# FitSNAP/FitSNAP

Hardware: AMD Instinct MI355X
Metric: training rows/sec through A^T A + solve, 1000000 x 128 fp64 in total over the GPUs (strong scaling) (higher is better)
Workload: dtype f64

## Files before the change

fitsnap_amd/csrc/fsnap_condest.h:

```cpp
#pragma once

#include <cmath>
#include <cstdint>
#include <vector>

namespace fsnap {

struct CondEstimate {
    double lambda_min = 0.0;
    int steps = 0;
};

inline double tridiag_lambda_max(const double* a, const double* b, int n) {
    double lo = a[0], hi = a[0];
    for (int i = 0; i < n; ++i) {
        const double r = (i > 0 ? std::fabs(b[i - 1]) : 0.0) + (i + 1 < n ? std::fabs(b[i]) : 0.0);
        if (a[i] - r < lo) lo = a[i] - r;
        if (a[i] + r > hi) hi = a[i] + r;
    }
    if (n == 1) return a[0];
    for (int it = 0; it < 200 && hi - lo > 4.0e-16 * std::fmax(std::fabs(hi), std::fabs(lo)); ++it) {
        const double x = 0.5 * (lo + hi);
        int above = 0;
        double d = 1.0;
        for (int i = 0; i < n; ++i) {
            const double off = i > 0 ? b[i - 1] * b[i - 1] : 0.0;
            d = (a[i] - x) - (i > 0 ? off / d : 0.0);
            if (d == 0.0) d = -1.0e-300;
            if (d > 0.0) ++above;
        }
        if (above > 0) lo = x; else hi = x;
    }
    return 0.5 * (lo + hi);
}

template <class ApplyInv>
CondEstimate lanczos_lambda_min(int n, ApplyInv&& apply_inv, int min_steps = 2, int max_steps = 8, double growth = 1.25,
                                double* theta_trace = nullptr) {
    CondEstimate out;
    if (n <= 0) return out;
    if (max_steps > 16) max_steps = 16;
    if (theta_trace)
        for (int j = 0; j < max_steps; ++j) theta_trace[j] = 0.0;
    std::vector<double> V((size_t)(max_steps + 1) * n), w(n);
    double al[16], be[16];
    uint64_t s = 0x9E3779B97F4A7C15ull;
    double nrm = 0.0;
    for (int i = 0; i < n; ++i) {
        s = s * 6364136223846793005ull + 1442695040888963407ull;
        const double u = (double)(int64_t)(s >> 11) * (1.0 / 9007199254740992.0);
        const double v = (u < 0.5 ? -1.0 : 1.0) * (0.25 + 0.75 * std::fabs(2.0 * u - 1.0));
        V[i] = v;
        nrm += v * v;
    }
    nrm = 1.0 / std::sqrt(nrm);
    for (int i = 0; i < n; ++i) V[i] *= nrm;
    double theta_prev = 0.0, theta = 0.0;
    for (int j = 0; j < max_steps; ++j) {
        double* vj = V.data() + (size_t)j * n;
        for (int i = 0; i < n; ++i) w[i] = vj[i];
        if (!apply_inv(w.data())) return CondEstimate{0.0, j + 1};
        double a = 0.0, chk = 0.0;
        for (int i = 0; i < n; ++i) {
            a += vj[i] * w[i];
            chk += w[i] * 0.0;
        }
        if (chk != 0.0 || !(a > 0.0)) return CondEstimate{0.0, j + 1};
        al[j] = a;
        out.steps = j + 1;
        theta = tridiag_lambda_max(al, be, j + 1);
        if (!(theta > 0.0) || !std::isfinite(theta)) return CondEstimate{0.0, j + 1};
        if (theta_trace) theta_trace[j] = theta;
        if (j + 1 >= min_steps && theta <= growth * theta_prev) break;
        if (j + 1 == max_steps) break;
        theta_prev = theta;
        for (int pass = 0; pass < 2; ++pass)
            for (int p = 0; p <= j; ++p) {
                const double* vp = V.data() + (size_t)p * n;
                double d = 0.0;
                for (int i = 0; i < n; ++i) d += vp[i] * w[i];
                for (int i = 0; i < n; ++i) w[i] -= d * vp[i];
            }
        double b = 0.0;
        for (int i = 0; i < n; ++i) b += w[i] * w[i];
        b = std::sqrt(b);
        if (!(b > 1.0e-14 * theta)) break;
        be[j] = b;
        double* vn = V.data() + (size_t)(j + 1) * n;
        const double ib = 1.0 / b;
        for (int i = 0; i < n; ++i) vn[i] = w[i] * ib;
    }
    out.lambda_min = 1.0 / theta;
    return out;
}

}
```

fitsnap_amd/csrc/fsnap_solve.cpp:

```cpp
#include <atomic>
#include <chrono>
#include <cstdio>
#include <cmath>
#include <cstdlib>
#include <cstdint>
#include <cstring>
#include <limits>
#include <mutex>
#include <thread>
#include <vector>

#include "../../include/fsnap_hip.h"
#include "fsnap_condest.h"

static thread_local double g_cond_info[4] = {0.0, 0.0, 0.0, 0.0};

extern "C" __attribute__((visibility("hidden"))) void fsnap_cond_note(double min_pivot, double lambda_min, int steps, int where) {
    g_cond_info[0] = min_pivot;
    g_cond_info[1] = lambda_min;
    g_cond_info[2] = (double)steps;
    g_cond_info[3] = (double)where;
}

extern "C" int fsnap_cond_info(double* info) {
// ... 155 lines not shown
    for (int c0 = ((je >> 5) + first_chunk) << 5; c0 < n; c0 += 32 * chunk_step) {
        const int cw = (n - c0 < 32) ? n - c0 : 32;
        const int i_end = (c0 + 32 < n) ? c0 + 32 : n;
        int i = je;
        if (cw == 32) {
            for (; i + 4 <= i_end; i += 4) {
                double* r0 = a + (size_t)i * n + c0;
                double* r1 = r0 + n;
                double* r2 = r1 + n;
                double* r3 = r2 + n;
                v8d y00 = *(const v8du*)(r0), y01 = *(const v8du*)(r0 + 8), y02 = *(const v8du*)(r0 + 16), y03 = *(const v8du*)(r0 + 24);
                v8d y10 = *(const v8du*)(r1), y11 = *(const v8du*)(r1 + 8), y12 = *(const v8du*)(r1 + 16), y13 = *(const v8du*)(r1 + 24);
                v8d y20 = *(const v8du*)(r2), y21 = *(const v8du*)(r2 + 8), y22 = *(const v8du*)(r2 + 16), y23 = *(const v8du*)(r2 + 24);
                v8d y30 = *(const v8du*)(r3), y31 = *(const v8du*)(r3 + 8), y32 = *(const v8du*)(r3 + 16), y33 = *(const v8du*)(r3 + 24);
                const double* uk = a + (size_t)jb * n;
                for (int k = 0; k < nk; ++k, uk += n) {
                    const v8d u0 = *(const v8du*)(uk + c0), u1 = *(const v8du*)(uk + c0 + 8);
                    const v8d u2 = *(const v8du*)(uk + c0 + 16), u3 = *(const v8du*)(uk + c0 + 24);
                    const double f0 = uk[i], f1 = uk[i + 1], f2 = uk[i + 2], f3 = uk[i + 3];
                    const v8d b0 = {f0, f0, f0, f0, f0, f0, f0, f0}, b1 = {f1, f1, f1, f1, f1, f1, f1, f1};
                    const v8d b2 = {f2, f2, f2, f2, f2, f2, f2, f2}, b3 = {f3, f3, f3, f3, f3, f3, f3, f3};
                    y00 -= b0 * u0; y01 -= b0 * u1; y02 -= b0 * u2; y03 -= b0 * u3;
                    y10 -= b1 * u0; y11 -= b1 * u1; y12 -= b1 * u2; y13 -= b1 * u3;
                    y20 -= b2 * u0; y21 -= b2 * u1; y22 -= b2 * u2; y23 -= b2 * u3;
                    y30 -= b3 * u0; y31 -= b3 * u1; y32 -= b3 * u2; y33 -= b3 * u3;
                }
                *(v8du*)(r0) = y00; *(v8du*)(r0 + 8) = y01; *(v8du*)(r0 + 16) = y02; *(v8du*)(r0 + 24) = y03;
                *(v8du*)(r1) = y10; *(v8du*)(r1 + 8) = y11; *(v8du*)(r1 + 16) = y12; *(v8du*)(r1 + 24) = y13;
                *(v8du*)(r2) = y20; *(v8du*)(r2 + 8) = y21; *(v8du*)(r2 + 16) = y22; *(v8du*)(r2 + 24) = y23;
                *(v8du*)(r3) = y30; *(v8du*)(r3 + 8) = y31; *(v8du*)(r3 + 16) = y32; *(v8du*)(r3 + 24) = y33;
            }
        }
        if (cw == 16) {
            for (; i + 4 <= i_end; i += 4) {
                double* r0 = a + (size_t)i * n + c0;
                double* r1 = r0 + n;
                double* r2 = r1 + n;
                double* r3 = r2 + n;
                v8d y00 = *(const v8du*)(r0), y01 = *(const v8du*)(r0 + 8);
                v8d y10 = *(const v8du*)(r1), y11 = *(const v8du*)(r1 + 8);
                v8d y20 = *(const v8du*)(r2), y21 = *(const v8du*)(r2 + 8);
                v8d y30 = *(const v8du*)(r3), y31 = *(const v8du*)(r3 + 8);
                const double* uk = a + (size_t)jb * n;
                for (int k = 0; k < nk; ++k, uk += n) {
                    const v8d u0 = *(const v8du*)(uk + c0), u1 = *(const v8du*)(uk + c0 + 8);
                    const double f0 = uk[i], f1 = uk[i + 1], f2 = uk[i + 2], f3 = uk[i + 3];
                    const v8d b0 = {f0, f0, f0, f0, f0, f0, f0, f0}, b1 = {f1, f1, f1, f1, f1, f1, f1, f1};
                    const v8d b2 = {f2, f2, f2, f2, f2, f2, f2, f2}, b3 = {f3, f3, f3, f3, f3, f3, f3, f3};
                    y00 -= b0 * u0; y01 -= b0 * u1;
                    y10 -= b1 * u0; y11 -= b1 * u1;
                    y20 -= b2 * u0; y21 -= b2 * u1;
                    y30 -= b3 * u0; y31 -= b3 * u1;
                }
                *(v8du*)(r0) = y00; *(v8du*)(r0 + 8) = y01;
                *(v8du*)(r1) = y10; *(v8du*)(r1 + 8) = y11;
                *(v8du*)(r2) = y20; *(v8du*)(r2 + 8) = y21;
                *(v8du*)(r3) = y30; *(v8du*)(r3 + 8) = y31;
            }
        }
        for (; i < i_end; ++i) {
            double* ri = a + (size_t)i * n + c0;
            const double* uk = a + (size_t)jb * n;
            for (int k = 0; k < nk; ++k, uk += n) axpy_neg(ri, uk + c0, uk[i], cw);
        }
    }
}

int chol_upper_rb(double* a, int n, double* min_piv2, int NBK) {
    double mp = std::numeric_limits<double>::infinity();
    for (int jb = 0; jb < n; jb += NBK) {
        const int je = (jb + NBK < n) ? jb + NBK : n;
        const int fail = chol_panel(a, n, jb, je, &mp);
        if (fail >= 0) {
            if (min_piv2) *min_piv2 = mp;
            return fail;
        }
        if (je < n) chol_trailing_chunks(a, n, jb, je, 0, 1);
    }
    if (min_piv2) *min_piv2 = mp;
    return -1;
}

FSNAP_CLONES void chol_solve_inv(const double* u, int n, double* x, double* inv) {
    for (int k = 0; k < n; ++k) inv[k] = 1.0 / u[(size_t)k * n + k];
    for (int k = 0; k < n; ++k) {
        const double* r = u + (size_t)k * n;
        x[k] *= inv[k];
        axpy_neg(x + k + 1, r + k + 1, x[k], n - 1 - k);
    }
    for (int i = n - 1; i >= 0; --i) {
        const double* r = u + (size_t)i * n;
        x[i] = (x[i] - dotv(r + i + 1, x + i + 1, n - 1 - i)) * inv[i];
    }
}
void chol_solve(const double* u, int n, double* x) {
    static thread_local vec inv;
    inv.resize(n);
    chol_solve_inv(u, n, x, inv.data());
}


#define LD8(p) (*reinterpret_cast<const v8du*>(p))
#define ST8(p, v) (*reinterpret_cast<v8du*>(p) = (v))
#define BC8(f) (v8d{(f), (f), (f), (f), (f), (f), (f), (f)})

FSNAP_INLINE void prefetch_g_rows(const double* G, int K, int r0, int r1) {
    if (r1 > K) r1 = K;
    for (int i = r0; i < r1; ++i) {
        const double* gi = G + (size_t)i * K;
        for (int j = i & ~7; j < K; j += 8) __builtin_prefetch(gi + j, 0, 2);
    }
}

FSNAP_INLINE void scaled_row(const double* G, const double* dsc, int K, int Kp, int i, double alpha, bool upper_only,
                             double* U, v8d& chk0, v8d& chk1, double& chk) {
    const v8d zero = {0, 0, 0, 0, 0, 0, 0, 0};
    const double* gi = G + (size_t)i * K;
    double* ui = U + (size_t)i * Kp;
    const double di = dsc[i];
    const v8d dv = {di, di, di, di, di, di, di, di};
    const int j0 = i & ~7;
    int j = 0;
    for (; j + 8 <= j0; j += 8) *(v8du*)(ui + j) = zero;
    if (upper_only && j + 8 <= K) {
        typedef long long v8l __attribute__((vector_size(64)));
        const v8l lanes = {0, 1, 2, 3, 4, 5, 6, 7};
        const v8l keep = (lanes + (long long)j) >= (long long)i;
        const v8d g0 = (v8d)((v8l)(*(const v8du*)(gi + j)) & keep);
        chk0 += g0 * zero;
        *(v8du*)(ui + j) = g0 * dv * *(const v8du*)(dsc + j);
        j += 8;
    }
    for (; j + 16 <= K; j += 16) {
        const v8d g0 = *(const v8du*)(gi + j), g1 = *(const v8du*)(gi + j + 8);
        chk0 += g0 * zero;
        chk1 += g1 * zero;
        *(v8du*)(ui + j) = g0 * dv * *(const v8du*)(dsc + j);
        *(v8du*)(ui + j + 8) = g1 * dv * *(const v8du*)(dsc + j + 8);
    }
    for (; j + 8 <= K; j += 8) {
        const v8d g0 = *(const v8du*)(gi + j);
        chk0 += g0 * zero;
        *(v8du*)(ui + j) = g0 * dv * *(const v8du*)(dsc + j);
    }
    for (; j < K; ++j) {
        const double gij = (upper_only && j < i) ? 0.0 : gi[j];
        ui[j] = gij * di * dsc[j];
        chk += gij * 0.0;
    }
    for (; j < Kp; ++j) ui[j] = 0.0;
    ui[i] = (gi[i] + alpha) * di * di;
}

template <bool RHS>
FSNAP_INLINE void left_update_8x16(const double* u, int n, int jb, int c0, v8d (&y)[16], double* z) {
    v8d zv = {0, 0, 0, 0, 0, 0, 0, 0};
    if (RHS) zv = LD8(z + jb);
    const double* uk = u;
    for (int k = 0; k < jb; ++k, uk += n) {
        const v8d u0 = LD8(uk + c0), u1 = LD8(uk + c0 + 8);
        const double* f = uk + jb;
#pragma unroll
        for (int r = 0; r < 8; ++r) {
            const v8d b = BC8(f[r]);
            y[2 * r] -= b * u0;
            y[2 * r + 1] -= b * u1;
        }
        if (RHS) {
            const v8d zk = BC8(z[k]);
            zv -= zk * LD8(f);
        }
    }
    if (RHS) ST8(z + jb, zv);
}

FSNAP_INLINE int fused_diag_block(double* u, int n, int jb, double* z, double* inv, double* mp) {
    const int c0 = jb & ~15, off = jb - c0;
    double* blk = u + (size_t)jb * n + c0;
    if (jb > 0) {
        v8d y[16];
#pragma unroll
        for (int r = 0; r < 8; ++r) {
            y[2 * r] = LD8(blk + (size_t)r * n);
            y[2 * r + 1] = LD8(blk + (size_t)r * n + 8);
        }
        left_update_8x16<true>(u, n, jb, c0, y, z);
#pragma unroll
        for (int r = 0; r < 8; ++r) {
            ST8(blk + (size_t)r * n, y[2 * r]);
            ST8(blk + (size_t)r * n + 8, y[2 * r + 1]);
        }
    }
    for (int j = 0; j < 8; ++j) {
        double* uj = blk + (size_t)j * n;
        const double d = uj[off + j];
        if (d < *mp) *mp = d;
        if (!(d > 0.0) || !std::isfinite(d)) return jb + j;
        const double r = std::sqrt(d), iv = 1.0 / r;
        inv[j] = iv;
        const v8d ivv = BC8(iv);
        const v8d s0 = LD8(uj) * ivv, s1 = LD8(uj + 8) * ivv;
        ST8(uj, s0);
        ST8(uj + 8, s1);
        uj[off + j] = r;
        const double zj = z[jb + j] * iv;
        z[jb + j] = zj;
        for (int i = j + 1; i < 8; ++i) {
            const double f = uj[off + i];
            z[jb + i] -= zj * f;
            if (f != 0.0) {
                double* ui = blk + (size_t)i * n;
                const v8d fv = BC8(f);
                v8d y0 = LD8(ui), y1 = LD8(ui + 8);
                y0 -= fv * s0;
                y1 -= fv * s1;
                ST8(ui, y0);
                ST8(ui + 8, y1);
            }
        }
    }
    return -1;
}

FSNAP_INLINE void fused_right_block(double* u, int n, int jb, int c0, const double* inv) {
    double* blk = u + (size_t)jb * n + c0;
    v8d y[16];
#pragma unroll
    for (int r = 0; r < 8; ++r) {
        y[2 * r] = LD8(blk + (size_t)r * n);
        y[2 * r + 1] = LD8(blk + (size_t)r * n + 8);
    }
    left_update_8x16<false>(u, n, jb, c0, y, nullptr);
    const double* fr = u + (size_t)jb * n + jb;
#pragma unroll
    for (int j = 0; j < 8; ++j) {
        const v8d ivv = BC8(inv[j]);
        y[2 * j] *= ivv;
        y[2 * j + 1] *= ivv;
#pragma unroll
        for (int i = j + 1; i < 8; ++i) {
            const double f = fr[(size_t)j * n + i];
            if (f != 0.0) {
                const v8d fv = BC8(f);
                y[2 * i] -= fv * y[2 * j];
                y[2 * i + 1] -= fv * y[2 * j + 1];
            }
        }
    }
#pragma unroll
    for (int r = 0; r < 8; ++r) {
        ST8(blk + (size_t)r * n, y[2 * r]);
        ST8(blk + (size_t)r * n + 8, y[2 * r + 1]);
    }
}

FSNAP_CLONES int fused_scale_chol(const double* G, const double* dsc, int K, int Kp, double alpha, bool upper_only,
                                  double* u, double* z, double* inv, double* min_piv2, double* chk_out) {
    const v8d zero = {0, 0, 0, 0, 0, 0, 0, 0};
    v8d chk0 = zero, chk1 = zero;
    double chk = 0.0;
    double mp = std::numeric_limits<double>::infinity();
    int fail = -1;
    for (int jb = 0; jb < Kp && fail < 0; jb += 8) {
        prefetch_g_rows(G, K, jb + 16, jb + 24);
        for (int i = jb; i < jb + 8; ++i) {
            if (i < K) {
                scaled_row(G, dsc, K, Kp, i, alpha, upper_only, u, chk0, chk1, chk);
            } else {
                double* ui = u + (size_t)i * Kp;
                for (int j = 0; j < Kp; ++j) ui[j] = 0.0;
                ui[i] = 1.0;
            }
        }
        fail = fused_diag_block(u, Kp, jb, z, inv + jb, &mp);
        if (fail >= 0) break;
        for (int c0 = (jb & ~15) + 16; c0 < Kp; c0 += 16) fused_right_block(u, Kp, jb, c0, inv + jb);
    }
    const v8d cs = chk0 + chk1;
    chk += ((cs[0] + cs[1]) + (cs[2] + cs[3])) + ((cs[4] + cs[5]) + (cs[6] + cs[7]));
    *chk_out = chk;
    *min_piv2 = mp;
    return fail;
}

FSNAP_CLONES bool jacobi_scale(const double* d, int K, double alpha, double* dsc) {
    typedef long long v8l __attribute__((vector_size(64)));
    const v8d zero = {0, 0, 0, 0, 0, 0, 0, 0};
    const v8d av = BC8(alpha), one = BC8(1.0);
    v8l good = {-1, -1, -1, -1, -1, -1, -1, -1};
    int i = 0;
    for (; i + 8 <= K; i += 8) {
        const v8d g = LD8(d + i) + av;
        good &= (g > zero) & (g - g == zero);
        ST8(dsc + i, one / __builtin_elementwise_sqrt(g));
    }
    bool ok = (good[0] & good[1] & good[2] & good[3] & good[4] & good[5] & good[6] & good[7]) != 0;
    for (; i < K; ++i) {
        const double g = d[i] + alpha;
        if (!(g > 0.0) || !std::isfinite(g)) ok = false;
        dsc[i] = 1.0 / std::sqrt(g);
    }
    return ok;
}

FSNAP_CLONES void chol_back_inv(const double* u, int n, double* x, const double* inv) {
    for (int i = n - 1; i >= 0; --i) {
        const double* r = u + (size_t)i * n;
        x[i] = (x[i] - dotv(r + i + 1, x + i + 1, n - 1 - i)) * inv[i];
    }
}

bool lu_solve(double* a, int n, double* b) {
    std::vector<int> piv(n);
    for (int j = 0; j < n; ++j) {
        int p = j;
        double mx = std::fabs(a[(size_t)j * n + j]);
        for (int i = j + 1; i < n; ++i) {
            double v = std::fabs(a[(size_t)i * n + j]);
            if (v > mx) {
                mx = v;
                p = i;
            }
        }
        if (!(mx > 0.0) || !std::isfinite(mx)) return false;
        if (p != j) {
            for (int k = 0; k < n; ++k) std::swap(a[(size_t)j * n + k], a[(size_t)p * n + k]);
            std::swap(b[j], b[p]);
        }
        const double inv = 1.0 / a[(size_t)j * n + j];
        for (int i = j + 1; i < n; ++i) {
            double f = a[(size_t)i * n + j] * inv;
            if (f == 0.0) continue;
            a[(size_t)i * n + j] = f;
            for (int k = j + 1; k < n; ++k) a[(size_t)i * n + k] -= f * a[(size_t)j * n + k];
            b[i] -= f * b[j];
        }
    }
    for (int i = n - 1; i >= 0; --i) {
        double s = b[i];
        for (int k = i + 1; k < n; ++k) s -= a[(size_t)i * n + k] * b[k];
        b[i] = s / a[(size_t)i * n + i];
    }
    return true;
}

void jacobi_eigh(double* a, int n, double* eval, double* v) {
    for (int i = 0; i < n; ++i)
        for (int j = 0; j < n; ++j) v[(size_t)i * n + j] = (i == j) ? 1.0 : 0.0;
    for (int sweep = 0; sweep < 60; ++sweep) {
        double off = 0.0, diag = 0.0;
        for (int i = 0; i < n; ++i) {
            diag += a[(size_t)i * n + i] * a[(size_t)i * n + i];
            for (int j = i + 1; j < n; ++j) off += a[(size_t)i * n + j] * a[(size_t)i * n + j];
        }
        if (off == 0.0 || off <= 1e-34 * diag) break;
        for (int p = 0; p < n - 1; ++p) {
            for (int q = p + 1; q < n; ++q) {
                const double apq = a[(size_t)p * n + q];
                if (apq == 0.0) continue;
                const double app = a[(size_t)p * n + p], aqq = a[(size_t)q * n + q];
                if (std::fabs(apq) <= 1e-18 * std::sqrt(std::fabs(app) * std::fabs(aqq))) {
                    a[(size_t)p * n + q] = a[(size_t)q * n + p] = 0.0;
                    continue;
                }
                const double theta = (aqq - app) / (2.0 * apq);
                const double t = (theta >= 0 ? 1.0 : -1.0) / (std::fabs(theta) + std::sqrt(theta * theta + 1.0));
                const double cs = 1.0 / std::sqrt(t * t + 1.0), sn = t * cs;
                for (int k = 0; k < n; ++k) {
                    const double akp = a[(size_t)k * n + p], akq = a[(size_t)k * n + q];
                    a[(size_t)k * n + p] = cs * akp - sn * akq;
                    a[(size_t)k * n + q] = sn * akp + cs * akq;
                }
                for (int k = 0; k < n; ++k) {
                    const double apk = a[(size_t)p * n + k], aqk = a[(size_t)q * n + k];
                    a[(size_t)p * n + k] = cs * apk - sn * aqk;
                    a[(size_t)q * n + k] = sn * apk + cs * aqk;
                }
                a[(size_t)p * n + q] = a[(size_t)q * n + p] = 0.0;
                double* vp = v + (size_t)p * n;
                double* vq = v + (size_t)q * n;
                for (int k = 0; k < n; ++k) {
                    const double x = vp[k], y = vq[k];
                    vp[k] = cs * x - sn * y;
                    vq[k] = sn * x + cs * y;
                }
            }
        }
    }
    for (int i = 0; i < n; ++i) eval[i] = a[(size_t)i * n + i];
}

void residual_dot2(const double* M, int n, const double* x, const double* rhs, double* r) {
    for (int i = 0; i < n; ++i) {
        const double* mi = M + (size_t)i * n;
        v4d s = {0, 0, 0, 0}, c = {0, 0, 0, 0};
        int k = 0;
        for (; k + 4 <= n; k += 4) {
            const v4d a = ld4(mi + k), b = ld4(x + k);
            const v4d p = a * b;
            v4d e;
            for (int t = 0; t < 4; ++t) e[t] = __builtin_fma(a[t], b[t], -p[t]);
            const v4d sn = s + p;
            const v4d bp = sn - s;
            const v4d err = (s - (sn - bp)) + (p - bp);
            s = sn;
            c += err + e;
        }
        double ss = 0.0, cc = 0.0;
        for (int t = 0; t < 4; ++t) {
            const double sn = ss + s[t];
            const double bp = sn - ss;
            cc += (ss - (sn - bp)) + (s[t] - bp) + c[t];
            ss = sn;
        }
        for (; k < n; ++k) {
            const double p = mi[k] * x[k];
            const double e = __builtin_fma(mi[k], x[k], -p);
            const double sn = ss + p;
            const double bp = sn - ss;
            cc += (ss - (sn - bp)) + (p - bp) + e;
            ss = sn;
        }
        const double t1 = rhs[i] - ss;
        r[i] = t1 - cc;
    }
}

struct Reduced {
    int n;
    std::vector<int> idx;
    vec M;
    vec rhs;
};

bool all_finite(const double* p, size_t n) {
    const v8d zero = {0, 0, 0, 0, 0, 0, 0, 0};
    v8d s0 = zero, s1 = zero, s2 = zero, s3 = zero;
    size_t i = 0;
    for (; i + 32 <= n; i += 32) {
        s0 += *(const v8du*)(p + i) * zero;
        s1 += *(const v8du*)(p + i + 8) * zero;
        s2 += *(const v8du*)(p + i + 16) * zero;
        s3 += *(const v8du*)(p + i + 24) * zero;
    }
    const v8d s = (s0 + s1) + (s2 + s3);
    double t = ((s[0] + s[1]) + (s[2] + s[3])) + ((s[4] + s[5]) + (s[6] + s[7]));
    for (; i < n; ++i) t += p[i] * 0.0;
    return t == 0.0;
}

int scaled_chol_solve(const vec& M, const vec& rhs, int n, vec& x, double* min_piv2, fsnap::CondEstimate* cond = nullptr) {
    vec d(n), y(n);
    static thread_local vec S;
    S.resize((size_t)n * n);
    for (int i = 0; i < n; ++i) {
        const double g = M[(size_t)i * n + i];
        if (!(g > 0.0)) {
            if (min_piv2) *min_piv2 = 0.0;
            return i;
        }
        d[i] = 1.0 / std::sqrt(g);
// ... 23 lines not shown
    return -1;
}

int eig_pinv_solve(const vec& M, const vec& rhs, int n, double rel_cut, double shift, vec& x) {
    vec a(M), ev(n), V((size_t)n * n);
    jacobi_eigh(a.data(), n, ev.data(), V.data());
    double lmax = 0.0;
    for (int i = 0; i < n; ++i) lmax = std::fmax(lmax, std::fabs(ev[i]));
    x.assign(n, 0.0);
    int rank = 0;
    for (int i = 0; i < n; ++i) {
        if (!(ev[i] > rel_cut * lmax)) continue;
        ++rank;
        const double* vi = V.data() + (size_t)i * n;
        long double s = 0.0L;
        for (int k = 0; k < n; ++k) s += (long double)vi[k] * rhs[k];
        const double coef = (double)(s / (long double)(ev[i] + shift));
        for (int k = 0; k < n; ++k) x[k] += coef * vi[k];
    }
    return rank;
}

FSNAP_CLONES int chol_panel_diag(double* a, int n, int jb, int je, double* mp) {
    for (int j = jb; j < je; ++j) {
        double* uj = a + (size_t)j * n;
        const double d = uj[j];
        if (d < *mp) *mp = d;
        if (!(d > 0.0) || !std::isfinite(d)) return j;
        const double r = std::sqrt(d), inv = 1.0 / r;
        uj[j] = r;
        for (int k = j + 1; k < je; ++k) uj[k] *= inv;
        for (int i = j + 1; i < je; ++i) {
            const double f = uj[i];
            double* ui = a + (size_t)i * n;
            for (int k = i; k < je; ++k) ui[k] -= f * uj[k];
        }
    }
    return -1;
}
FSNAP_CLONES void chol_panel_tails(double* a, int n, int jb, int je, int first_chunk, int chunk_step) {
    for (int c0 = je + 32 * first_chunk; c0 < n; c0 += 32 * chunk_step) {
        const int cw = (n - c0 < 32) ? n - c0 : 32;
        for (int j = jb; j < je; ++j) {
            double* uj = a + (size_t)j * n;
            const double inv = 1.0 / uj[j];
            for (int k = 0; k < cw; ++k) uj[c0 + k] *= inv;
            for (int i = j + 1; i < je; ++i) axpy_neg(a + (size_t)i * n + c0, uj + c0, uj[i], cw);
        }
    }
}

int chol_upper_rb_mt(double* a, int n, double* min_piv2, int NBK, int nt) {
    struct Shared {
        std::atomic<int> arrived{0};
        std::atomic<int> phase{0};
        std::atomic<int> fail{-1};
        double mp = std::numeric_limits<double>::infinity();
    } sh;
    auto barrier = [&](int& local_phase) {
        ++local_phase;
        if (sh.arrived.fetch_add(1, std::memory_order_acq_rel) + 1 == nt) {
            sh.arrived.store(0, std::memory_order_relaxed);
            sh.phase.store(local_phase, std::memory_order_release);
        } else {
            int spins = 0;
            while (sh.phase.load(std::memory_order_acquire) != local_phase) {
#if defined(__x86_64__)
                __builtin_ia32_pause();
#endif
                if (++spins > 4096) {
                    std::this_thread::yield();
                    spins = 0;
                }
            }
        }
    };
    auto body = [&](int t) {
        int ph = 0;
        for (int jb = 0; jb < n; jb += NBK) {
            const int je = (jb + NBK < n) ? jb + NBK : n;
            if (t == 0) {
                const int f = chol_panel_diag(a, n, jb, je, &sh.mp);
                if (f >= 0) sh.fail.store(f, std::memory_order_relaxed);
            }
            barrier(ph);
            if (sh.fail.load(std::memory_order_relaxed) >= 0) return;
            if (je < n) {
                chol_panel_tails(a, n, jb, je, t, nt);
                barrier(ph);
                chol_trailing_chunks(a, n, jb, je, t, nt);
            }
            barrier(ph);
        }
    };
    std::vector<std::thread> th;
    th.reserve(nt - 1);
    for (int t = 1; t < nt; ++t) th.emplace_back(body, t);
    body(0);
    for (auto& x : th) x.join();
    if (min_piv2) *min_piv2 = sh.mp;
    return sh.fail.load();
}

int chol_variant_env() {
    static const int forced = [] {
        const char* e = std::getenv("FSNAP_CHOL_VARIANT");
        return e ? std::atoi(e) : 0;
    }();
    return forced;
}
int chol_nbk_env() {
    static const int nbk_env = [] {
        const char* e = std::getenv("FSNAP_CHOL_NBK");
        return e ? std::atoi(e) : 0;
    }();
    return nbk_env;
}

bool use_fused_finish(int n) { return chol_variant_env() == 0 && chol_nbk_env() <= 0 && n >= 48 && n <= 256 && (n & 15) == 0; }

int fast_chol(double* u, int n, double* mp2) {
    const int forced = chol_variant_env();
    const int nbk_env = chol_nbk_env();
    if (forced == 1) return chol_upper(u, n, mp2);
    if (forced == 2) return chol_upper_blocked(u, n, mp2, 64);
    if (forced == 3 || n >= 48) {
        const int nbk = nbk_env > 0 ? nbk_env : (n <= 256 ? 8 : 32);
        static const int nt_env = [] {
            const char* e = std::getenv("FSNAP_CHOL_THREADS");
            return e ? std::atoi(e) : 0;
        }();
        static const int nt_auto = [] {
            auto quota = [](const char* path, bool v2) -> bool {
                FILE* f = std::fopen(path, "r");
                if (!f) return false;
                char buf[64] = {0};
                const bool got = std::fgets(buf, sizeof buf, f) != nullptr;
                std::fclose(f);
                if (!got) return false;
                return v2 ? std::strncmp(buf, "max", 3) != 0 : std::atol(buf) > 0;
            };
            if (quota("/sys/fs/cgroup/cpu.max", true) || quota("/sys/fs/cgroup/cpu/cpu.cfs_quota_us", false)) return 1;
            const unsigned hc = std::thread::hardware_concurrency();
            return (int)(hc >= 8 ? 8 : (hc > 0 ? hc : 1));
        }();
        int nt = nt_env > 0 ? nt_env : nt_auto;
        if (nt > n / 160) nt = n / 160;
        if (nt > 1) return chol_upper_rb_mt(u, n, mp2, nbk, nt);
        return chol_upper_rb(u, n, mp2, nbk);
    }
    return chol_upper(u, n, mp2);
}

}

namespace {
struct PhaseTotals {
    static const int MAXP = 16;
    std::mutex mu;
    const char* name[MAXP];
    double us[MAXP];
    long calls[MAXP];
    int n = 0;
    void add(const char* what, double t) {
        std::lock_guard<std::mutex> lk(mu);
        int p = 0;
        while (p < n && std::strcmp(name[p], what) != 0) ++p;
        if (p == n) {
            if (n == MAXP) return;
            name[n] = what;
            us[n] = 0.0;
            calls[n] = 0;
            ++n;
        }
        us[p] += t;
        ++calls[p];
    }
    void print() {
        std::lock_guard<std::mutex> lk(mu);
        for (int p = 0; p < n; ++p)
            std::fprintf(stderr, "[fsnap_solve] total %-26s %8ld calls %12.1f us  mean %9.2f us\n", name[p], calls[p], us[p],
                         us[p] / (double)calls[p]);
    }
};
PhaseTotals& phase_totals() {
    static PhaseTotals* t = [] {
        static PhaseTotals totals;
        std::atexit([] { phase_totals().print(); });
        return &totals;
    }();
    return *t;
}
struct PhaseTimer {
    int mode;
    std::chrono::steady_clock::time_point t0;
    static int env_mode() {
        static const int m = [] {
            const char* e = std::getenv("FSNAP_SOLVE_TIMING");
            if (!e) return 0;
            return std::atoi(e) == 2 ? 2 : 1;
        }();
        return m;
    }
    PhaseTimer() : mode(env_mode()) {
        if (mode) t0 = std::chrono::steady_clock::now();
    }
    void lap(const char* what) {
        if (!mode) return;
        const auto t1 = std::chrono::steady_clock::now();
        const double us = std::chrono::duration<double, std::micro>(t1 - t0).count();
        if (mode == 2) phase_totals().add(what, us);
        else std::fprintf(stderr, "[fsnap_solve] %-14s %9.1f us\n", what, us);
        t0 = mode == 2 ? std::chrono::steady_clock::now() : t1;
    }
};
}

extern "C" int fsnap_solve_diag(int kind, double param, int64_t K64, const double* G, const double* c, const double* diag,
                                double* beta, int* rank_out, double* rcond_est);
extern "C" int fsnap_solve_diag_upper(int kind, double param, int64_t K64, const double* G, const double* c, const double* diag,
                                      double* beta, int* rank_out, double* rcond_est);
namespace {
int solve_impl(int kind, double param, int64_t K64, const double* G, const double* c, const double* diag, double* beta,
               int* rank_out, double* rcond_est, bool upper_only, const void* owner = nullptr, unsigned long long generation = 0);
}

extern "C" __attribute__((visibility("hidden"))) int fsnap_host_chol_upper(double* a, int n, double* min_piv) {
    return fast_chol(a, n, min_piv);
}

extern "C" __attribute__((visibility("hidden"))) double fsnap_gen_eig_max(const double* M, const double* N, int k) {
    if (k <= 0 || !all_finite(M, (size_t)k * k) || !all_finite(N, (size_t)k * k)) return -1.0;
    vec U(N, N + (size_t)k * k), C((size_t)k * k);
    for (int i = 0; i < k; ++i)
        for (int j = 0; j < i; ++j) U[(size_t)i * k + j] = 0.0;
    double mp = 0.0;
    if (chol_upper(U.data(), k, &mp) >= 0) return -1.0;
    vec T(M, M + (size_t)k * k);
    auto forward_columns = [&](vec& X) {
        for (int i = 0; i < k; ++i) {
            const double inv = 1.0 / U[(size_t)i * k + i];
            for (int c = 0; c < k; ++c) {
                double sacc = X[(size_t)i * k + c];
                for (int l = 0; l < i; ++l) sacc -= U[(size_t)l * k + i] * X[(size_t)l * k + c];
                X[(size_t)i * k + c] = sacc * inv;
            }
        }
    };
    forward_columns(T);
    for (int i = 0; i < k; ++i)
        for (int j = 0; j < k; ++j) C[(size_t)i * k + j] = T[(size_t)j * k + i];
    forward_columns(C);
    for (int i = 0; i < k; ++i)
        for (int j = i + 1; j < k; ++j) C[(size_t)i * k + j] = C[(size_t)j * k + i] = 0.5 * (C[(size_t)i * k + j] + C[(size_t)j * k + i]);
    vec ta((size_t)k), tb((size_t)k), hv((size_t)k), hp((size_t)k);
    for (int j = 0; j + 2 < k; ++j) {
        const int m = k - j - 1;
        double nrm2 = 0.0;
        for (int i = 0; i < m; ++i) {
            hv[i] = C[(size_t)(j + 1 + i) * k + j];
            nrm2 += hv[i] * hv[i];
        }
        const double nrm = std::sqrt(nrm2);
        ta[j] = C[(size_t)j * k + j];
        tb[j] = nrm;
        if (!(nrm > 0.0)) continue;
        hv[0] += hv[0] >= 0.0 ? nrm : -nrm;
        double vn = 0.0;
        for (int i = 0; i < m; ++i) vn += hv[i] * hv[i];
        vn = 1.0 / std::sqrt(vn);
        for (int i = 0; i < m; ++i) hv[i] *= vn;
        double vp = 0.0;
        for (int r = 0; r < m; ++r) {
            double acc = 0.0;
            for (int c = 0; c < m; ++c) acc += C[(size_t)(j + 1 + r) * k + j + 1 + c] * hv[c];
            hp[r] = acc;
            vp += hv[r] * acc;
        }
        for (int r = 0; r < m; ++r) hp[r] -= vp * hv[r];
        for (int r = 0; r < m; ++r)
            for (int c = 0; c < m; ++c) C[(size_t)(j + 1 + r) * k + j + 1 + c] -= 2.0 * (hv[r] * hp[c] + hp[r] * hv[c]);
    }
    if (k >= 2) {
        ta[k - 2] = C[(size_t)(k - 2) * k + k - 2];
        tb[k - 2] = C[(size_t)(k - 1) * k + k - 2];
    }
    ta[k - 1] = C[(size_t)(k - 1) * k + k - 1];
    const double theta = fsnap::tridiag_lambda_max(ta.data(), tb.data(), k);
    return theta > 0.0 && std::isfinite(theta) ? theta : -1.0;
}

extern "C" int fsnap_solve(int kind, double param, int64_t K64, const double* G, const double* c, double* beta,
                           int* rank_out, double* rcond_est) {
    return fsnap_solve_diag(kind, param, K64, G, c, nullptr, beta, rank_out, rcond_est);
}

extern "C" __attribute__((visibility("hidden"))) int fsnap_solve_diag(int kind, double param, int64_t K64, const double* G,
                                                                      const double* c, const double* diag, double* beta,
                                                                      int* rank_out, double* rcond_est) {
    return solve_impl(kind, param, K64, G, c, diag, beta, rank_out, rcond_est, false);
}

extern "C" __attribute__((visibility("hidden"))) int fsnap_solve_diag_upper(int kind, double param, int64_t K64, const double* G,
                                                                            const double* c, const double* diag, double* beta,
                                                                            int* rank_out, double* rcond_est) {
    return solve_impl(kind, param, K64, G, c, diag, beta, rank_out, rcond_est, true);
}

extern "C" __attribute__((visibility("hidden"))) int fsnap_solve_diag_tagged(int kind, double param, int64_t K64, const double* G,
                                                                             const double* c, const double* diag, double* beta,
                                                                             int* rank_out, double* rcond_est, int upper,
                                                                             const void* owner, unsigned long long generation) {
    return solve_impl(kind, param, K64, G, c, diag, beta, rank_out, rcond_est, upper != 0, owner, generation);
}

namespace {
int solve_impl(int kind, double param, int64_t K64, const double* G, const double* c, const double* diag, double* beta,
               int* rank_out, double* rcond_est, bool upper_only, const void* owner, unsigned long long generation) {
    PhaseTimer timer;
    if (!G || !c || !beta || K64 <= 0 || K64 > (1 << 20)) return FSNAP_E_ARG;
    if (kind < FSNAP_SOLVE_CHOL || kind > FSNAP_SOLVE_RIDGE_INV_PROBE) return FSNAP_E_ARG;
    const bool probe = kind >= FSNAP_SOLVE_LSTSQ_PROBE;
    if (kind == FSNAP_SOLVE_LSTSQ_PROBE) kind = FSNAP_SOLVE_LSTSQ;
    if (kind == FSNAP_SOLVE_RIDGE_PROBE) kind = FSNAP_SOLVE_RIDGE;
    if (kind == FSNAP_SOLVE_RIDGE_INV_PROBE) kind = FSNAP_SOLVE_RIDGE_INV;
    const int K = (int)K64;
    if (!std::isfinite(param)) return FSNAP_NUM_NONFINITE;
    const double alpha = (kind == FSNAP_SOLVE_RIDGE || kind == FSNAP_SOLVE_RIDGE_INV) ? param : 0.0;
    const double eps = std::numeric_limits<double>::epsilon();
    timer.lap("finite check");

    {
        int Kp = (K >= 48 && (K & 15) != 0) ? ((K + 15) & ~15) : K;
        if (Kp >= 384 && (Kp & 127) == 0) Kp += 32;
        static thread_local vec U, dsc, z;
        static thread_local struct { const void* owner; unsigned long long gen; int K; double alpha, mp2, piv, lam; } held = {nullptr, 0, 0, 0.0, 0.0, 0.0, 0.0};
        if (owner && held.owner == owner && held.gen == generation && held.K == K && held.alpha == alpha &&
            U.size() == (size_t)Kp * Kp) {
            bool fin = true;
            for (int i = 0; i < K; ++i) {
                z[i] = c[i] * dsc[i];
                fin = fin && (c[i] - c[i] == 0.0);
            }
            if (fin) {
                for (int i = K; i < Kp; ++i) z[i] = 0.0;
                chol_solve(U.data(), Kp, z.data());
                for (int i = 0; i < K; ++i) beta[i] = z[i] * dsc[i];
                timer.lap("tri solves (factor reused)");
                if (all_finite(beta, K)) {
                    if (rank_out) *rank_out = K;
                    if (rcond_est) *rcond_est = held.mp2;
                    fsnap_cond_note(held.piv, held.lam, 0, 0);
                    return FSNAP_OK;
                }
            }
        }
        held.owner = nullptr;
        const bool fused = use_fused_finish(Kp);
        if (fused) prefetch_g_rows(G, K, 0, 16);
        static thread_local vec uinv;
        U.resize((size_t)Kp * Kp);
        dsc.resize(Kp);
        z.resize(Kp);
        bool ok = true;
        double chk = 0.0;
        if (fused) {
            uinv.resize(Kp);
            if (!diag)
                for (int i = 0; i < K; ++i) dsc[i] = G[(size_t)i * K + i];
            ok = jacobi_scale(diag ? diag : dsc.data(), K, alpha, dsc.data());
            bool fin = true;
            for (int i = 0; i < K; ++i) {
                z[i] = c[i] * dsc[i];
                fin = fin && (c[i] - c[i] == 0.0);
            }
            for (int i = K; i < Kp; ++i) z[i] = 0.0;
            if (!fin) chk = std::numeric_limits<double>::quiet_NaN();
        } else {
            for (int i = 0; i < K && ok; ++i) {
                const double g = (diag ? diag[i] : G[(size_t)i * K + i]) + alpha;
                if (!(g > 0.0) || !std::isfinite(g)) ok = false;
                else dsc[i] = 1.0 / std::sqrt(g);
                chk += c[i] * 0.0;
            }
        }
        timer.lap("diag scale");
        if (ok) {
            double mp2 = 0.0;
            bool fact_ok;
            if (fused) {
                double gchk = 0.0;
                fact_ok = (chk == 0.0) &&
                          fused_scale_chol(G, dsc.data(), K, Kp, alpha, upper_only, U.data(), z.data(), uinv.data(), &mp2, &gchk) < 0 &&
                          gchk == 0.0;
                timer.lap("fused finish");
            } else {
                const v8d zero = {0, 0, 0, 0, 0, 0, 0, 0};
                v8d chk0 = zero, chk1 = zero;
                for (int i = 0; i < K; ++i) {
                    if (i + 2 < K) {
                        const double* gn = G + (size_t)(i + 2) * K;
                        for (int jp = (i + 2) & ~7; jp < K; jp += 8) __builtin_prefetch(gn + jp, 0, 0);
                    }
                    scaled_row(G, dsc.data(), K, Kp, i, alpha, upper_only, U.data(), chk0, chk1, chk);
                }
                for (int i = K; i < Kp; ++i) {
                    double* ui = U.data() + (size_t)i * Kp;
                    for (int j = 0; j < Kp; ++j) ui[j] = 0.0;
                    ui[i] = 1.0;
                }
                const v8d cs = chk0 + chk1;
                chk += ((cs[0] + cs[1]) + (cs[2] + cs[3])) + ((cs[4] + cs[5]) + (cs[6] + cs[7]));
                timer.lap("scale/build");
                fact_ok = (chk == 0.0) && fast_chol(U.data(), Kp, &mp2) < 0;
                timer.lap("cholesky");
            }
            fsnap::CondEstimate ce;
            bool cond_ok = true;
            if (fact_ok && mp2 > 1.0e-3 && kind == FSNAP_SOLVE_LSTSQ) {
                const double* Up = U.data();
                ce = fsnap::lanczos_lambda_min(Kp, [Up, Kp](double* v) {
                    chol_solve(Up, Kp, v);
                    return true;
                });
                cond_ok = ce.lambda_min > 64.0 * K * eps;
                timer.lap("cond estimate");
            }
            if (fact_ok && mp2 > 1.0e-3 && cond_ok) {
                const double piv = mp2;
                if (ce.steps && ce.lambda_min < mp2) mp2 = ce.lambda_min;
                fsnap_cond_note(piv, ce.lambda_min, ce.steps, 0);
                if (fused) {
                    chol_back_inv(U.data(), Kp, z.data(), uinv.data());
                } else {
                    for (int i = 0; i < K; ++i) z[i] = c[i] * dsc[i];
                    for (int i = K; i < Kp; ++i) z[i] = 0.0;
                    chol_solve(U.data(), Kp, z.data());
                }
                for (int i = 0; i < K; ++i) beta[i] = z[i] * dsc[i];
                timer.lap(fused ? "back sweep" : "tri solves");
                if (all_finite(beta, K)) {
                    if (rank_out) *rank_out = K;
                    if (rcond_est) *rcond_est = mp2;
                    if (owner) {
                        held.owner = owner;
                        held.gen = generation;
                        held.K = K;
                        held.alpha = alpha;
                        held.mp2 = mp2;
                        held.piv = piv;
                        held.lam = ce.lambda_min;
                    }
                    return FSNAP_OK;
                }
            }
        }
    }

    static thread_local vec Gfull;
    if (upper_only) {
        Gfull.resize((size_t)K * K);
        for (int i = 0; i < K; ++i)
            for (int j = i; j < K; ++j) Gfull[(size_t)i * K + j] = Gfull[(size_t)j * K + i] = G[(size_t)i * K + j];
        G = Gfull.data();
    }
    if (!all_finite(G, (size_t)K * K) || !all_finite(c, K)) return FSNAP_NUM_NONFINITE;
    static thread_local Reduced R;
    R.idx.clear();
    R.idx.reserve(K);
    for (int j = 0; j < K; ++j) {
        const double gjj = G[(size_t)j * K + j] + alpha;
        if (gjj == 0.0 && kind != FSNAP_SOLVE_CHOL && kind != FSNAP_SOLVE_RIDGE_INV) continue;
        R.idx.push_back(j);
    }
    const int n = R.n = (int)R.idx.size();
    for (int j = 0; j < K; ++j) beta[j] = 0.0;
    if (rank_out) *rank_out = 0;
    if (rcond_est) *rcond_est = 0.0;
    if (n == 0) return FSNAP_OK;
    R.M.resize((size_t)n * n);
    R.rhs.resize(n);
    for (int i = 0; i < n; ++i) {
        R.rhs[i] = c[R.idx[i]];
        for (int j = 0; j < n; ++j) {
            const double gij = 0.5 * (G[(size_t)R.idx[i] * K + R.idx[j]] + G[(size_t)R.idx[j] * K + R.idx[i]]);
            R.M[(size_t)i * n + j] = gij + ((i == j) ? alpha : 0.0);
        }
    }

    vec x;
    double mp2 = 0.0;
    fsnap::CondEstimate ce;
    const int fail = scaled_chol_solve(R.M, R.rhs, n, x, &mp2, kind == FSNAP_SOLVE_LSTSQ ? &ce : nullptr);
    const double piv = mp2;
    if (fail < 0 && ce.steps && ce.lambda_min < mp2) mp2 = ce.lambda_min;
    fsnap_cond_note(piv, ce.lambda_min, ce.steps, 0);
    if (rcond_est) *rcond_est = mp2;
    const double piv_tol = 64.0 * n * eps;
    const bool chol_ok = (fail < 0) && (mp2 > piv_tol);

    if (chol_ok) {
        for (int i = 0; i < n; ++i) beta[R.idx[i]] = x[i];
        if (rank_out) *rank_out = n;
        return all_finite(beta, K) ? FSNAP_OK : FSNAP_NUM_NONFINITE;
    }

    if (probe) {
        if (rank_out) *rank_out = -1;
        return FSNAP_OK;
    }
    switch (kind) {
        case FSNAP_SOLVE_CHOL:
            return FSNAP_NUM_NOT_SPD;
        case FSNAP_SOLVE_LSTSQ: {
            double cut = param > 0 ? param * param : 0.0;
            const double floor_cut = 4.0 * n * eps;
            if (cut < floor_cut) cut = floor_cut;
            const int rk = eig_pinv_solve(R.M, R.rhs, n, cut, 0.0, x);
            for (int i = 0; i < n; ++i) beta[R.idx[i]] = x[i];
            if (rank_out) *rank_out = rk;
            return all_finite(beta, K) ? FSNAP_OK : FSNAP_NUM_NONFINITE;
        }
        case FSNAP_SOLVE_RIDGE: {
            const int rk = eig_pinv_solve(R.M, R.rhs, n, 4.0 * n * eps, 0.0, x);
            for (int i = 0; i < n; ++i) beta[R.idx[i]] = x[i];
            if (rank_out) *rank_out = rk;
            return all_finite(beta, K) ? FSNAP_OK : FSNAP_NUM_NONFINITE;
        }
        case FSNAP_SOLVE_RIDGE_INV: {
            vec a(R.M), b(R.rhs);
            if (!lu_solve(a.data(), n, b.data())) return FSNAP_NUM_SINGULAR;
            for (int i = 0; i < n; ++i) beta[R.idx[i]] = b[i];
            if (rank_out) *rank_out = n;
            return all_finite(beta, K) ? FSNAP_OK : FSNAP_NUM_NONFINITE;
        }
    }
    return FSNAP_E_ARG;
}

}

extern "C" int fsnap_lasso_gram(int64_t K64, const double* Q, const double* q, double y_norm2, double l1_reg, int64_t max_iter,
                                double tol, double* w, int64_t* n_iter_out, double* gap_out) {
    if (!Q || !q || !w || K64 <= 0 || K64 > (1 << 20) || max_iter < 1 || !(l1_reg >= 0.0) || !(tol >= 0.0)) return FSNAP_E_ARG;
    const int n = (int)K64;
    if (!all_finite(Q, (size_t)n * n) || !all_finite(q, n) || !std::isfinite(y_norm2)) return FSNAP_NUM_NONFINITE;
    vec H((size_t)n, 0.0);
    for (int i = 0; i < n; ++i) {
        if (w[i] == 0.0) continue;
        const double* Qi = Q + (size_t)i * n;
        for (int j = 0; j < n; ++j) H[j] += w[i] * Qi[j];
    }
    const double d_w_tol = tol;
    const double gap_tol = tol * y_norm2;
    double gap = gap_tol + 1.0;
    int64_t it = 0;
    for (it = 0; it < max_iter; ++it) {
        double w_max = 0.0, d_w_max = 0.0;
        for (int i = 0; i < n; ++i) {
            const double* __restrict__ Qi = Q + (size_t)i * n;
            const double Qii = Qi[i];
            if (Qii == 0.0) continue;
            const double w_old = w[i];
            double* __restrict__ h = H.data();
            if (w_old != 0.0)
                for (int j = 0; j < n; ++j) h[j] -= w_old * Qi[j];
            const double t = q[i] - h[i];
            const double mag = std::fabs(t) - l1_reg;
            const double w_new = mag > 0.0 ? std::copysign(mag, t) / Qii : 0.0;
            w[i] = w_new;
            if (w_new != 0.0)
                for (int j = 0; j < n; ++j) h[j] += w_new * Qi[j];
            d_w_max = std::fmax(d_w_max, std::fabs(w_new - w_old));
            w_max = std::fmax(w_max, std::fabs(w_new));
        }
        if (w_max == 0.0 || d_w_max / w_max < d_w_tol || it == max_iter - 1) {
            double q_dot_w = 0.0, wHw = 0.0, l1 = 0.0, dual = 0.0;
            for (int i = 0; i < n; ++i) {
                q_dot_w += w[i] * q[i];
// ... 24 lines not shown
```

Measured before the change: 3.085 billion.

## Speed up Lanczos condition estimate with blocked solves and fused first RHS

Replaces the generic Lanczos condition estimator with a specialized path. The starting vector is cached per thread. Its forward substitution is folded into the fused Cholesky as a second right-hand side, so the first step needs only a back solve. Later steps use a blocked triangular apply with precomputed inverse diagonals, and the Ritz value comes from a Newton iteration instead of bisection. The aim is to cut CPU time in the small K=128 solve tail, at the cost of more code paths and a slightly different convergence check.

```diff
diff --git a/fitsnap_amd/csrc/fsnap_condest.h b/fitsnap_amd/csrc/fsnap_condest.h
--- a/fitsnap_amd/csrc/fsnap_condest.h
+++ b/fitsnap_amd/csrc/fsnap_condest.h
@@ -1,5 +1,6 @@
 #pragma once
 
+#include <chrono>
 #include <cmath>
 #include <cstdint>
 #include <vector>
@@ -9,6 +10,15 @@
 struct CondEstimate {
     double lambda_min = 0.0;
     int steps = 0;
+};
+
+struct CondPhases {
+    double apply_us = 0.0;
+    double reorth_us = 0.0;
+    double ritz_us = 0.0;
+    static double now() {
+        return std::chrono::duration<double, std::micro>(std::chrono::steady_clock::now().time_since_epoch()).count();
+    }
 };
 
 inline double tridiag_lambda_max(const double* a, const double* b, int n) {
@@ -34,9 +44,46 @@
     return 0.5 * (lo + hi);
 }
 
+inline double tridiag_lambda_max_newton(const double* a, const double* b, int n) {
+    if (n == 1) return a[0];
+    if (n > 16) return tridiag_lambda_max(a, b, n);
+    double hi = a[0], amax = std::fabs(a[0]);
+    for (int i = 0; i < n; ++i) {
+        const double r = (i > 0 ? std::fabs(b[i - 1]) : 0.0) + (i + 1 < n ? std::fabs(b[i]) : 0.0);
+        if (a[i] + r > hi) hi = a[i] + r;
+        if (std::fabs(a[i]) + r > amax) amax = std::fabs(a[i]) + r;
+    }
+    if (!(amax > 0.0) || !std::isfinite(amax)) return tridiag_lambda_max(a, b, n);
+    int e = 0;
+    std::frexp(amax, &e);
+    const double sc = std::ldexp(1.0, -e);
+    double as[16], b2[16];
+    for (int i = 0; i < n; ++i) as[i] = a[i] * sc;
+    for (int i = 0; i + 1 < n; ++i) {
+        const double bs = b[i] * sc;
+        b2[i] = bs * bs;
+    }
+    double x = hi * sc;
+    for (int it = 0; it < 100; ++it) {
+        double p0 = 1.0, p1 = as[0] - x, d0 = 0.0, d1 = -1.0;
+        for (int i = 1; i < n; ++i) {
+            const double t = as[i] - x;
+            const double p2 = t * p1 - b2[i - 1] * p0;
+            const double d2 = t * d1 - p1 - b2[i - 1] * d0;
+            p0 = p1; p1 = p2;
+            d0 = d1; d1 = d2;
+        }
+        const double dx = p1 / d1;
+        if (!(dx > 0.0)) return x * std::ldexp(1.0, e);
+        x -= dx;
+        if (dx <= 2.3e-16 * std::fabs(x)) return x * std::ldexp(1.0, e);
+    }
+    return tridiag_lambda_max(a, b, n);
+}
+
 template <class ApplyInv>
 CondEstimate lanczos_lambda_min(int n, ApplyInv&& apply_inv, int min_steps = 2, int max_steps = 8, double growth = 1.25,
-                                double* theta_trace = nullptr) {
+                                double* theta_trace = nullptr, CondPhases* ph = nullptr) {
     CondEstimate out;
     if (n <= 0) return out;
     if (max_steps > 16) max_steps = 16;
@@ -59,7 +106,14 @@
     for (int j = 0; j < max_steps; ++j) {
         double* vj = V.data() + (size_t)j * n;
         for (int i = 0; i < n; ++i) w[i] = vj[i];
-        if (!apply_inv(w.data())) return CondEstimate{0.0, j + 1};
+        double t0 = 0.0, t1 = 0.0, t2 = 0.0;
+        if (ph) t0 = CondPhases::now();
+        const bool applied = apply_inv(w.data());
+        if (ph) {
+            t1 = CondPhases::now();
+            ph->apply_us += t1 - t0;
+        }
+        if (!applied) return CondEstimate{0.0, j + 1};
         double a = 0.0, chk = 0.0;
         for (int i = 0; i < n; ++i) {
             a += vj[i] * w[i];
@@ -71,6 +125,10 @@
         theta = tridiag_lambda_max(al, be, j + 1);
         if (!(theta > 0.0) || !std::isfinite(theta)) return CondEstimate{0.0, j + 1};
         if (theta_trace) theta_trace[j] = theta;
+        if (ph) {
+            t2 = CondPhases::now();
+            ph->ritz_us += t2 - t1;
+        }
         if (j + 1 >= min_steps && theta <= growth * theta_prev) break;
         if (j + 1 == max_steps) break;
         theta_prev = theta;
@@ -89,6 +147,7 @@
         double* vn = V.data() + (size_t)(j + 1) * n;
         const double ib = 1.0 / b;
         for (int i = 0; i < n; ++i) vn[i] = w[i] * ib;
+        if (ph) ph->reorth_us += CondPhases::now() - t2;
     }
     out.lambda_min = 1.0 / theta;
     return out;
diff --git a/fitsnap_amd/csrc/fsnap_solve.cpp b/fitsnap_amd/csrc/fsnap_solve.cpp
--- a/fitsnap_amd/csrc/fsnap_solve.cpp
+++ b/fitsnap_amd/csrc/fsnap_solve.cpp
@@ -331,10 +331,11 @@
     ui[i] = (gi[i] + alpha) * di * di;
 }
 
-template <bool RHS>
-FSNAP_INLINE void left_update_8x16(const double* u, int n, int jb, int c0, v8d (&y)[16], double* z) {
-    v8d zv = {0, 0, 0, 0, 0, 0, 0, 0};
+template <bool RHS, bool RHS2 = false>
+FSNAP_INLINE void left_update_8x16(const double* u, int n, int jb, int c0, v8d (&y)[16], double* z, double* z2 = nullptr) {
+    v8d zv = {0, 0, 0, 0, 0, 0, 0, 0}, zv2 = zv;
     if (RHS) zv = LD8(z + jb);
+    if (RHS2) zv2 = LD8(z2 + jb);
     const double* uk = u;
     for (int k = 0; k < jb; ++k, uk += n) {
         const v8d u0 = LD8(uk + c0), u1 = LD8(uk + c0 + 8);
@@ -349,11 +350,17 @@
             const v8d zk = BC8(z[k]);
             zv -= zk * LD8(f);
         }
+        if (RHS2) {
+            const v8d zk2 = BC8(z2[k]);
+            zv2 -= zk2 * LD8(f);
+        }
     }
     if (RHS) ST8(z + jb, zv);
-}
-
-FSNAP_INLINE int fused_diag_block(double* u, int n, int jb, double* z, double* inv, double* mp) {
+    if (RHS2) ST8(z2 + jb, zv2);
+}
+
+template <bool RHS2>
+FSNAP_INLINE int fused_diag_block(double* u, int n, int jb, double* z, double* z2, double* inv, double* mp) {
     const int c0 = jb & ~15, off = jb - c0;
     double* blk = u + (size_t)jb * n + c0;
     if (jb > 0) {
@@ -363,7 +370,7 @@
             y[2 * r] = LD8(blk + (size_t)r * n);
             y[2 * r + 1] = LD8(blk + (size_t)r * n + 8);
         }
-        left_update_8x16<true>(u, n, jb, c0, y, z);
+        left_update_8x16<true, RHS2>(u, n, jb, c0, y, z, z2);
 #pragma unroll
         for (int r = 0; r < 8; ++r) {
             ST8(blk + (size_t)r * n, y[2 * r]);
@@ -384,9 +391,15 @@
         uj[off + j] = r;
         const double zj = z[jb + j] * iv;
         z[jb + j] = zj;
+        double zj2 = 0.0;
+        if (RHS2) {
+            zj2 = z2[jb + j] * iv;
+            z2[jb + j] = zj2;
+        }
         for (int i = j + 1; i < 8; ++i) {
             const double f = uj[off + i];
             z[jb + i] -= zj * f;
+            if (RHS2) z2[jb + i] -= zj2 * f;
             if (f != 0.0) {
                 double* ui = blk + (size_t)i * n;
                 const v8d fv = BC8(f);
@@ -433,8 +446,9 @@
     }
 }
 
-FSNAP_CLONES int fused_scale_chol(const double* G, const double* dsc, int K, int Kp, double alpha, bool upper_only,
-                                  double* u, double* z, double* inv, double* min_piv2, double* chk_out) {
+template <bool RHS2>
+FSNAP_INLINE int fused_scale_chol_body(const double* G, const double* dsc, int K, int Kp, double alpha, bool upper_only,
+                                       double* u, double* z, double* z2, double* inv, double* min_piv2, double* chk_out) {
     const v8d zero = {0, 0, 0, 0, 0, 0, 0, 0};
     v8d chk0 = zero, chk1 = zero;
     double chk = 0.0;
@@ -451,7 +465,7 @@
                 ui[i] = 1.0;
             }
         }
-        fail = fused_diag_block(u, Kp, jb, z, inv + jb, &mp);
+        fail = fused_diag_block<RHS2>(u, Kp, jb, z, z2, inv + jb, &mp);
         if (fail >= 0) break;
         for (int c0 = (jb & ~15) + 16; c0 < Kp; c0 += 16) fused_right_block(u, Kp, jb, c0, inv + jb);
     }
@@ -460,6 +474,14 @@
     *chk_out = chk;
     *min_piv2 = mp;
     return fail;
+}
+FSNAP_CLONES int fused_scale_chol(const double* G, const double* dsc, int K, int Kp, double alpha, bool upper_only,
+                                  double* u, double* z, double* inv, double* min_piv2, double* chk_out) {
+    return fused_scale_chol_body<false>(G, dsc, K, Kp, alpha, upper_only, u, z, nullptr, inv, min_piv2, chk_out);
+}
+FSNAP_CLONES int fused_scale_chol_rhs2(const double* G, const double* dsc, int K, int Kp, double alpha, bool upper_only,
+                                       double* u, double* z, double* z2, double* inv, double* min_piv2, double* chk_out) {
+    return fused_scale_chol_body<true>(G, dsc, K, Kp, alpha, upper_only, u, z, z2, inv, min_piv2, chk_out);
 }
 
 FSNAP_CLONES bool jacobi_scale(const double* d, int K, double alpha, double* dsc) {
@@ -486,6 +508,57 @@
     for (int i = n - 1; i >= 0; --i) {
         const double* r = u + (size_t)i * n;
         x[i] = (x[i] - dotv(r + i + 1, x + i + 1, n - 1 - i)) * inv[i];
+    }
+}
+
+#define HSUM8(v) ((((v)[0] + (v)[1]) + ((v)[2] + (v)[3])) + (((v)[4] + (v)[5]) + ((v)[6] + (v)[7])))
+FSNAP_CLONES void chol_apply_inv(const double* u, int n, double* x, const double* inv, bool forward) {
+    if (forward)
+        for (int k0 = 0; k0 < n; k0 += 8) {
+            const double* r0 = u + (size_t)k0 * n;
+            for (int r = 0; r < 8; ++r) {
+                double t = x[k0 + r];
+                for (int q = 0; q < r; ++q) t -= r0[(size_t)q * n + k0 + r] * x[k0 + q];
+                x[k0 + r] = t * inv[k0 + r];
+            }
+            v8d y[8];
+#pragma unroll
+            for (int r = 0; r < 8; ++r) y[r] = BC8(x[k0 + r]);
+            for (int c = k0 + 8; c < n; c += 8) {
+                v8d xv = LD8(x + c);
+#pragma unroll
+                for (int r = 0; r < 8; ++r) xv -= y[r] * LD8(r0 + (size_t)r * n + c);
+                ST8(x + c, xv);
+            }
+        }
+    for (int i0 = n - 8; i0 >= 0; i0 -= 8) {
+        const double* r0 = u + (size_t)i0 * n;
+        const v8d zero = {0, 0, 0, 0, 0, 0, 0, 0};
+        v8d a[8];
+#pragma unroll
+        for (int r = 0; r < 8; ++r) a[r] = zero;
+        for (int c = i0 + 8; c < n; c += 8) {
+            const v8d xv = LD8(x + c);
+#pragma unroll
+            for (int r = 0; r < 8; ++r) a[r] += LD8(r0 + (size_t)r * n + c) * xv;
+        }
+        double s[8];
+#pragma unroll
+        for (int r = 0; r < 8; ++r) s[r] = HSUM8(a[r]);
+        for (int r = 7; r >= 0; --r) {
+            const double* ur = r0 + (size_t)r * n + i0;
+            double t = x[i0 + r] - s[r];
+            for (int c = 7; c > r; --c) t -= ur[c] * x[i0 + c];
+            x[i0 + r] = t * inv[i0 + r];
+        }
+    }
+}
+
+FSNAP_CLONES void chol_fwd_inv(const double* u, int n, double* x, const double* inv) {
+    for (int k = 0; k < n; ++k) {
+        const double* r = u + (size_t)k * n;
+        x[k] *= inv[k];
+        axpy_neg(x + k + 1, r + k + 1, x[k], n - 1 - k);
     }
 }
 
@@ -815,6 +888,89 @@
     return chol_upper(u, n, mp2);
 }
 
+int condest_variant_env() {
+    static const int forced = [] {
+        const char* e = std::getenv("FSNAP_CONDEST_VARIANT");
+        return e ? std::atoi(e) : 0;
+    }();
+    return forced;
+}
+
+const double* condest_start(int n) {
+    static thread_local vec v0;
+    static thread_local int held_n = 0;
+    if (held_n == n) return v0.data();
+    v0.resize(n);
+    uint64_t s = 0x9E3779B97F4A7C15ull;
+    double nrm = 0.0;
+    for (int i = 0; i < n; ++i) {
+        s = s * 6364136223846793005ull + 1442695040888963407ull;
+        const double u = (double)(int64_t)(s >> 11) * (1.0 / 9007199254740992.0);
+        const double v = (u < 0.5 ? -1.0 : 1.0) * (0.25 + 0.75 * std::fabs(2.0 * u - 1.0));
+        v0[i] = v;
+        nrm += v * v;
+    }
+    nrm = 1.0 / std::sqrt(nrm);
+    for (int i = 0; i < n; ++i) v0[i] *= nrm;
+    held_n = n;
+    return v0.data();
+}
+
+FSNAP_CLONES void condest_fast(const double* u, int n, const double* inv, const double* v0, const double* y0, double* V,
+                               fsnap::CondPhases* ph, fsnap::CondEstimate* res) {
+    const int min_steps = 2, max_steps = 8;
+    const double growth = 1.25;
+    res->lambda_min = 0.0;
+    res->steps = 0;
+    double* w = V + (size_t)(max_steps + 1) * n;
+    double al[16], be[16];
+    std::memcpy(V, v0, (size_t)n * sizeof(double));
+    double theta_prev = 0.0, theta = 0.0;
+    for (int j = 0; j < max_steps; ++j) {
+        const double* vj = V + (size_t)j * n;
+        double t0 = 0.0, t1 = 0.0, t2 = 0.0;
+        if (ph) t0 = fsnap::CondPhases::now();
+        if (j == 0 && y0 && inv) {
+            std::memcpy(w, y0, (size_t)n * sizeof(double));
+            chol_apply_inv(u, n, w, inv, false);
+        } else {
+            std::memcpy(w, vj, (size_t)n * sizeof(double));
+            if (inv) chol_apply_inv(u, n, w, inv, true);
+            else chol_solve(u, n, w);
+        }
+        if (ph) {
+            t1 = fsnap::CondPhases::now();
+            ph->apply_us += t1 - t0;
+        }
+        const double a = dotv(vj, w, n);
+        res->steps = j + 1;
+        if (!all_finite(w, (size_t)n) || !(a > 0.0)) return;
+        al[j] = a;
+        theta = fsnap::tridiag_lambda_max_newton(al, be, j + 1);
+        if (!(theta > 0.0) || !std::isfinite(theta)) return;
+        if (ph) {
+            t2 = fsnap::CondPhases::now();
+            ph->ritz_us += t2 - t1;
+        }
+        if (j + 1 >= min_steps && theta <= growth * theta_prev) break;
+        if (j + 1 == max_steps) break;
+        theta_prev = theta;
+        for (int pass = 0; pass < 2; ++pass)
+            for (int p = 0; p <= j; ++p) {
+                const double* vp = V + (size_t)p * n;
+                axpy_neg(w, vp, dotv(vp, w, n), n);
+            }
+        const double b = std::sqrt(dotv(w, w, n));
+        if (!(b > 1.0e-14 * theta)) break;
+        be[j] = b;
+        double* vn = V + (size_t)(j + 1) * n;
+        const double ib = 1.0 / b;
+        for (int i = 0; i < n; ++i) vn[i] = w[i] * ib;
+        if (ph) ph->reorth_us += fsnap::CondPhases::now() - t2;
+    }
+    res->lambda_min = 1.0 / theta;
+}
+
 }
 
 namespace {
@@ -876,6 +1032,13 @@
         else std::fprintf(stderr, "[fsnap_solve] %-14s %9.1f us\n", what, us);
         t0 = mode == 2 ? std::chrono::steady_clock::now() : t1;
     }
+    void note(const char* what, double value) {
+        if (!mode) return;
+        if (mode == 2) {
+            phase_totals().add(what, value);
+            t0 = std::chrono::steady_clock::now();
+        } else std::fprintf(stderr, "[fsnap_solve]   %-12s %9.1f\n", what, value);
+    }
 };
 }
 
@@ -1021,7 +1184,19 @@
         held.owner = nullptr;
         const bool fused = use_fused_finish(Kp);
         if (fused) prefetch_g_rows(G, K, 0, 16);
-        static thread_local vec uinv;
+        static thread_local vec uinv, cws;
+        const bool ce_fast = kind == FSNAP_SOLVE_LSTSQ && condest_variant_env() == 0;
+        const bool ce_blocked = ce_fast && Kp >= 48 && Kp <= 256 && (Kp & 15) == 0;
+        const double* cv0 = nullptr;
+        double* cy0 = nullptr;
+        if (ce_fast) {
+            cws.resize((size_t)11 * Kp);
+            cv0 = condest_start(Kp);
+            if (ce_blocked) {
+                cy0 = cws.data() + (size_t)10 * Kp;
+                std::memcpy(cy0, cv0, (size_t)Kp * sizeof(double));
+            }
+        }
         U.resize((size_t)Kp * Kp);
         dsc.resize(Kp);
         z.resize(Kp);
@@ -1054,7 +1229,8 @@
             if (fused) {
                 double gchk = 0.0;
                 fact_ok = (chk == 0.0) &&
-                          fused_scale_chol(G, dsc.data(), K, Kp, alpha, upper_only, U.data(), z.data(), uinv.data(), &mp2, &gchk) < 0 &&
+                          (ce_blocked ? fused_scale_chol_rhs2(G, dsc.data(), K, Kp, alpha, upper_only, U.data(), z.data(), cy0, uinv.data(), &mp2, &gchk)
+                               : fused_scale_chol(G, dsc.data(), K, Kp, alpha, upper_only, U.data(), z.data(), uinv.data(), &mp2, &gchk)) < 0 &&
                           gchk == 0.0;
                 timer.lap("fused finish");
             } else {
@@ -1077,17 +1253,34 @@
                 timer.lap("scale/build");
                 fact_ok = (chk == 0.0) && fast_chol(U.data(), Kp, &mp2) < 0;
                 timer.lap("cholesky");
+                if (fact_ok && ce_blocked) {
+                    uinv.resize(Kp);
+                    for (int k = 0; k < Kp; ++k) uinv[k] = 1.0 / U[(size_t)k * Kp + k];
+                    chol_fwd_inv(U.data(), Kp, cy0, uinv.data());
+                }
             }
             fsnap::CondEstimate ce;
             bool cond_ok = true;
             if (fact_ok && mp2 > 1.0e-3 && kind == FSNAP_SOLVE_LSTSQ) {
                 const double* Up = U.data();
-                ce = fsnap::lanczos_lambda_min(Kp, [Up, Kp](double* v) {
-                    chol_solve(Up, Kp, v);
-                    return true;
-                });
+                fsnap::CondPhases phs;
+                fsnap::CondPhases* ph = timer.mode ? &phs : nullptr;
+                if (ce_fast) {
+                    condest_fast(Up, Kp, ce_blocked ? uinv.data() : nullptr, cv0, cy0, cws.data(), ph, &ce);
+                } else {
+                    ce = fsnap::lanczos_lambda_min(Kp, [Up, Kp](double* v) {
+                        chol_solve(Up, Kp, v);
+                        return true;
+                    }, 2, 8, 1.25, nullptr, ph);
+                }
                 cond_ok = ce.lambda_min > 64.0 * K * eps;
                 timer.lap("cond estimate");
+                if (ph) {
+                    timer.note("ce: S^-1 apply", phs.apply_us);
+                    timer.note("ce: ritz value", phs.ritz_us);
+                    timer.note("ce: reorth", phs.reorth_us);
+                    timer.note("ce: steps", (double)ce.steps);
+                }
             }
             if (fact_ok && mp2 > 1.0e-3 && cond_ok) {
                 const double piv = mp2;
```

New measurement: 3.091 billion, median of 3. No clear change (+0.2%).
